# buggyyang/CDC_compression

Measured on AMD Instinct MI355X. Metric: decoded images/sec at 256x256, 500-step x-param, higher is better.
Workload: dtype f32 (f16x2 split products)

## Files before the change

### cdc_compression_amd/_lib.py

```python
import ctypes
import os
import subprocess

import numpy as np

_HERE = os.path.dirname(os.path.abspath(__file__))
LIB_PATH = os.environ.get("CDC_HIP_LIB") or os.path.join(_HERE, "libcdc_hip.so")

CDC_MEM_HOST, CDC_MEM_DEVICE = 0, 1
CDC_PRED_X, CDC_PRED_NOISE, CDC_PRED_NOISE_XTREE, CDC_PRED_V = 0, 1, 2, 3
CDC_CLIP_NONE, CDC_CLIP_ALL, CDC_CLIP_HALF = 0, 1, 2
CDC_MAX_LEVELS = 8
CDC_ELEM_F32, CDC_ELEM_U8 = 0, 1
CDC_FILL_EDGE, CDC_FILL_ZERO = 0, 1
CDC_METRIC_PSNR, CDC_METRIC_MSSSIM = 1, 2
CDC_TRACE_X0, CDC_TRACE_XT, CDC_TRACE_U8 = 1, 2, 4

_f = ctypes.POINTER(ctypes.c_float)
_i = ctypes.c_int
_vp = ctypes.c_void_p


class UnetConfig(ctypes.Structure):
    _fields_ = [("dim", ctypes.c_int32), ("channels", ctypes.c_int32),
# ... 162 lines not shown
    L.cdc_randn_host.argtypes = [u64p, _i, ctypes.c_int64, ctypes.c_uint32, ctypes.c_float, _vp]
    L.cdc_philox4x32_10.argtypes = [ctypes.POINTER(ctypes.c_uint32)] * 3
    i32p = ctypes.POINTER(ctypes.c_int32)
    L.cdc_set_noise_frames.argtypes = [H, i32p, _i]
    L.cdc_randn_framed.argtypes = [H, u64p, i32p, _i, _i, _i, _i, ctypes.c_uint32, ctypes.c_float, _vp, _i, _vp]
    L.cdc_randn_framed_host.argtypes = [u64p, i32p, _i, _i, _i, _i, ctypes.c_uint32, ctypes.c_float, _vp]
    L.cdc_tile_gather.argtypes = [H, _vp, _vp, i32p] + [_i] * 8 + [_vp]
    L.cdc_tile_blend.argtypes = [H, _vp, _vp, i32p, _i, i32p, _i, _vp] + [_i] * 14 + [_vp]
    L.cdc_prof_enable.argtypes = [H, _i]
    L.cdc_prof_name.argtypes = [_i]
    L.cdc_prof_name.restype = ctypes.c_char_p
    L.cdc_prof_get.argtypes = [H, _i, ctypes.POINTER(ctypes.c_double),
                               ctypes.POINTER(ctypes.c_int64), ctypes.POINTER(ctypes.c_double),
                               ctypes.POINTER(ctypes.c_double)]
    L.cdc_prof_reset.argtypes = [H]
    L.cdc_prof_num_ops.argtypes = [H]
    L.cdc_prof_op.argtypes = [H, _i, ctypes.POINTER(ctypes.c_char_p), ctypes.POINTER(ctypes.c_double),
                              ctypes.POINTER(ctypes.c_int64), ctypes.POINTER(ctypes.c_double)]
    L.cdc_op_conv2d.argtypes = [H, _vp, _vp, _vp, _vp] + [_i] * 9 + [_vp, _vp, _i, _vp, _vp]
    L.cdc_op_conv_transpose2d.argtypes = [H, _vp, _vp, _vp, _vp] + [_i] * 5
    L.cdc_op_chan_layernorm.argtypes = [H, _vp, _vp, _vp, _vp, _i, _i, _i]
    L.cdc_op_chan_layernorm_ex.argtypes = [H, _vp, _i, _vp, _vp, _i, _vp, _vp, _i, _vp, _vp, _vp, _i, _i, _i]
    L.cdc_op_ln_form.argtypes = [H, _i, _i, _i, _i, _i] + [ctypes.POINTER(_i)] * 4
    L.cdc_op_sum_slices.argtypes = [H, _vp, _i, _vp, _i, ctypes.c_longlong]
    L.cdc_op_linear_attention.argtypes = [H] + [_vp] * 7 + [_i] * 4
    L.cdc_op_stress.argtypes = [H, _i]
    L.cdc_op_stress_result.argtypes = [H, ctypes.POINTER(ctypes.c_int64), ctypes.POINTER(ctypes.c_int64)]
    L.cdc_probe_mfma_f16.argtypes = [_i, _i, _i, ctypes.POINTER(ctypes.c_double)]
    L.cdc_probe_hbm_copy.argtypes = [_i, ctypes.c_size_t, _i, ctypes.POINTER(ctypes.c_double)]
    _lib = L
# ... 11 lines not shown
           "cdc_entropy_encode", "cdc_entropy_peek", "cdc_entropy_set_limit", "cdc_entropy_decode", "cdc_get_range_faults",
           "cdc_get_nonfinite_results", "cdc_set_schedule_v", "cdc_probe_mfma_f16", "cdc_probe_hbm_copy",
           "cdc_op_stress", "cdc_op_stress_result", "cdc_enable_vbr", "cdc_set_bitrate_scale", "cdc_entropy_peek_bitrate_scale",
           "cdc_padded_size", "cdc_frame_pad", "cdc_frame_crop", "cdc_entropy_set_image_scale", "cdc_entropy_encode_image",
           "cdc_entropy_peek_image_size", "cdc_decode_seeded", "cdc_randn", "cdc_randn_host", "cdc_philox4x32_10",
           "cdc_distortion", "cdc_lpips_create", "cdc_lpips", "cdc_simple_encoder_create", "cdc_simple_ctxdec_create", "cdc_op_gdn",
           "cdc_op_gdn_workgroups", "cdc_op_chan_layernorm_ex", "cdc_op_ln_form", "cdc_op_sum_slices",
           "cdc_set_solver", "cdc_decode_solver", "cdc_solver_step", "cdc_op_solver_update", "cdc_op_ddim_update",
           "cdc_repeat_images", "cdc_decode_samples", "cdc_sample_moments", "cdc_sample_select",
           "cdc_set_trace", "cdc_trace_info", "cdc_trace_read", "cdc_op_trace_tap",
           "cdc_rate_map", "cdc_distortion_map", "cdc_set_rdo", "cdc_entropy_rate_sweep", "cdc_op_rdo_quantize",
           "cdc_price_cells", "cdc_set_rdo_map", "cdc_op_rdo_quantize_map",
           "cdc_set_noise_frames", "cdc_randn_framed", "cdc_randn_framed_host", "cdc_tile_gather", "cdc_tile_blend",
           "cdc_entropy_set_segments", "cdc_entropy_peek_segments", "cdc_entropy_decode_window",
           "cdc_entropy_set_hyper_groups", "cdc_entropy_peek_hyper_groups",
           "cdc_entropy_peek_partial", "cdc_entropy_decode_partial", "cdc_segment_mask"]


def handle_status(handle):
    if handle is None:
        return {"arith": None, "range_faults": 0, "nonfinite_results": 0}
    L = lib()
    return {"arith": int(L.cdc_get_arith(handle)), "range_faults": int(L.cdc_get_range_faults(handle)),
            "nonfinite_results": int(L.cdc_get_nonfinite_results(handle))}


def check(handle, rc):
    if rc != 0:
        msg = lib().cdc_last_error(handle)
        msg = msg.decode() if msg else ""
        if "must be multiples of" in msg:
# ... 90 lines not shown
```

### cdc_compression_amd/csrc/cdc_api.hip

```cpp
#include "cdc_state.h"
#include "rng.h"

namespace cdcapi {

std::string g_create_err;

int fail(cdc_handle *h, int code, const char *fmt, ...) {
    char buf[1024];
    va_list ap;
    va_start(ap, fmt);
    vsnprintf(buf, sizeof buf, fmt, ap);
    va_end(ap);
    if (h) h->err = buf; else g_create_err = buf;
    return code;
}

hipEvent_t get_event(cdc_handle *h) {
    if (!h->ev_free.empty()) { hipEvent_t e = h->ev_free.back(); h->ev_free.pop_back(); return e; }
    hipEvent_t e = nullptr;
    (void)hipEventCreate(&e);
    return e;
}

int resolve_pending(cdc_handle *h) {
// ... 38 lines not shown
        if (rc) return rc;
    }
    return CDC_OK;
}

int run_pre(cdc_handle *h, hipStream_t st) {
    for (const Op &op : h->pre_ops) {
        int rc = run_op(h, op, h->pB, st);
        if (rc) return rc;
    }
    return CDC_OK;
}

int run_unet(cdc_handle *h, hipStream_t st, int step, bool skip_combine) {
    for (const Op &op : h->ops) {
        if (skip_combine && op.get<CombineArgs>()) continue;
        int rc;
        if (op.get<TembArgs>() && (step >= 0 || step == -2)) {
            CopyArgs c = {h->d_shift_tab.p + (step >= 0 ? (size_t)step * h->shift_bs : 0), 0, h->shift, h->shift_bs, h->shift_bs};
            if (step == -2) { c.step = h->d_step; c.step_stride = h->shift_bs; }
            Op cop(op.prof, c, op.flops, op.bytes);
            cop.id = op.id;
            rc = run_op(h, cop, h->pB, st);
        } else {
            rc = run_op(h, op, h->pB, st);
        }
        if (rc) return rc;
    }
    return CDC_OK;
}
// ... 106 lines not shown
    return !no_guard && (h->arith == CDC_ARITH_F16X2 || h->in_retry);
}
int arm_range_guard(cdc_handle *h, hipStream_t st, bool always) {
    if (!always && !guard_enabled(h)) return CDC_OK;
    if (!h->d_fault) { void *p = nullptr; HIP_TRY(h, hipMalloc(&p, sizeof(int))); h->d_fault = (int *)p; h->weight_allocs.push_back(p); }
    HIP_TRY(h, hipMemsetAsync(h->d_fault, 0, sizeof(int), st));
    return CDC_OK;
}
int range_check(cdc_handle *h, const std::vector<GuardBuf> &bufs, int B, hipStream_t st) {
    if (!guard_enabled(h)) return CDC_OK;
    for (const GuardBuf &g : bufs)
        if (g.p && g.n > 0) HIP_TRY(h, cdc::nonfinite_launch(g.p, g.bs, g.n, B, h->d_fault, st));
    int fault = 0;
    HIP_TRY(h, hipMemcpyAsync(&fault, h->d_fault, sizeof(int), hipMemcpyDeviceToHost, st));
    HIP_TRY(h, hipStreamSynchronize(st));
    if (!fault) return CDC_OK;
    if (h->in_retry || h->arith != CDC_ARITH_F16X2) {
        ++h->nonfinite_results;
        if (h->in_retry) h->retry_futile = true;
        return CDC_OK;
    }
    ++h->range_faults;
    static bool warned = false;
    if (!warned) {
        warned = true;
        fprintf(stderr, "cdc_hip: a value left the fp16 range of CDC_ARITH_F16X2; the call is repeated in CDC_ARITH_BF16X3 and the handle stays "
                        "in that (slower, full-range) arithmetic -- see cdc_get_range_faults()\n");
    }
    int rc = cdc_set_arith(h, CDC_ARITH_BF16X3);
    return rc ? rc : kRangeRetry;
}

static int run_compressor(cdc_handle *h, const float *x, size_t n, int B, int mem, hipStream_t st) {
    int rc;
    if ((rc = stage_rate(h, nullptr, B, st))) return rc;
    if ((rc = copy_in(h, h->in_x, x, n, mem, st))) return rc;
    if ((rc = arm_range_guard(h, st, false))) return rc;
    h->prof_now = true;
    if ((rc = run_ops(h, h->pB, st))) return rc;
    std::vector<GuardBuf> outs;
    for (const Act &a : h->dec_outs) outs.push_back({a.p, a.bs(), (long long)a.C * a.H * a.W});
    return range_check(h, outs, B, st);
}

}

extern "C" {

const char *cdc_version(void) { return "cdc_hip 0.9 (gfx950; fp32-class convolutions from split fp16 / bf16 operands on the matrix cores)"; }

const char *cdc_last_error(const cdc_handle *h) { return h ? h->err.c_str() : g_create_err.c_str(); }

int cdc_create(const cdc_unet_config *cfg, int device, cdc_handle **out) {
    if (!cfg || !out) return fail(nullptr, CDC_ERR_INVALID, "null argument");
    if (cfg->dim <= 0 || cfg->n_dim_mults < 1 || cfg->n_dim_mults > CDC_MAX_LEVELS ||
        cfg->n_context_dim_mults < 0 || cfg->n_context_dim_mults > CDC_MAX_LEVELS || cfg->channels < 1)
        return fail(nullptr, CDC_ERR_INVALID, "bad cdc_unet_config");
// ... 3 lines not shown
    h->device = device;
    h->out_dim = cfg->out_dim > 0 ? cfg->out_dim : cfg->channels;
    h->dims.push_back(cfg->channels);
    for (int i = 0; i < cfg->n_dim_mults; ++i) h->dims.push_back(cfg->dim * cfg->dim_mults[i]);
    h->context_dims.push_back(cfg->context_channels);
    for (int i = 0; i < cfg->n_context_dim_mults; ++i)
        h->context_dims.push_back(cfg->dim * cfg->context_dim_mults[i]);
    h->n_res = cfg->n_dim_mults;
    build_manifest(h.get());
    *out = h.release();
    return CDC_OK;
}

void cdc_destroy(cdc_handle *h) {
    if (!h) return;
    if (!h->own_stream) { delete h; return; }
    (void)hipSetDevice(h->device);
    (void)hipDeviceSynchronize();
    free_program(h);
    free_pool(&h->weight_allocs);
    h->d_tab.release();
    h->d_tab_v.release();
    h->d_time_steps.release();
    h->d_shift_tab.release();
    h->seeds.dev.release();
    h->frames.dev.release();
    h->tile_meta.dev.release();
    h->d_stab.release();
    h->d_hist.release();
    h->d_rep_stage.release();
// ... 6 lines not shown
    for (hipEvent_t e : h->ev_free) (void)hipEventDestroy(e);
    if (h->gev_in) (void)hipEventDestroy(h->gev_in);
    if (h->gev_out) (void)hipEventDestroy(h->gev_out);
    if (h->graph_exec) (void)hipGraphExecDestroy(h->graph_exec);
    if (h->ev0) (void)hipEventDestroy(h->ev0);
    if (h->ev1) (void)hipEventDestroy(h->ev1);
    if (h->own_stream) (void)hipStreamDestroy(h->own_stream);
    delete h;
}

int cdc_set_arith(cdc_handle *h, int mode) {
    if (!h) return CDC_ERR_INVALID;
    if (mode != CDC_ARITH_BF16X3 && mode != CDC_ARITH_F16X2) return fail(h, CDC_ERR_INVALID, "arith mode %d", mode);
    if (mode != h->arith) {
        if (h->own_stream) { (void)hipSetDevice(h->device); (void)hipDeviceSynchronize(); }
        free_program(h);
        h->arith = mode;
    }
    return CDC_OK;
}

int cdc_get_arith(const cdc_handle *h) { return h ? h->arith : CDC_ERR_INVALID; }
int cdc_get_range_faults(const cdc_handle *h) { return h ? h->range_faults : CDC_ERR_INVALID; }
int cdc_get_nonfinite_results(const cdc_handle *h) { return h ? h->nonfinite_results : CDC_ERR_INVALID; }

int cdc_enable_vbr(cdc_handle *h) {
    if (!h) return CDC_ERR_INVALID;
    if (h->kind == HandleKind::Unet) return fail(h, CDC_ERR_INVALID, "variable bitrate needs a context-decoder, encoder or hyper-decoder handle");
    if (h->simple)
        return fail(h, CDC_ERR_INVALID, "variable bitrate: SimpleCompressor has no working VBR form in the reference");
// ... 826 lines not shown
}

int cdc_ddim_step(cdc_handle *h, const float *x_in, int i, const float *const *ctx, int n_ctx,
                  const float *noise, float eta, float *x_out, int B, int H, int W, int pred_mode,
                  int clip, int mem, void *stream) {
    if (!h) return CDC_ERR_INVALID;
    return no_throw(h, [&] { return sampler_step(h, false, x_in, noise, eta, i, ctx, n_ctx, x_out, nullptr, B, H, W, pred_mode, clip, mem, stream); });
}

int cdc_solver_step(cdc_handle *h, const float *x_in, const float *x0_prev_in, int i, const float *const *ctx, int n_ctx, float *x_out,
                    float *x0_out, int B, int H, int W, int pred_mode, int clip, int mem, void *stream) {
    if (!h) return CDC_ERR_INVALID;
    return no_throw(h, [&] { return sampler_step(h, true, x_in, x0_prev_in, 0.f, i, ctx, n_ctx, x_out, x0_out, B, H, W, pred_mode, clip, mem, stream); });
}

static int decode_impl(cdc_handle *h, const float *init, float gamma, const uint64_t *seeds, float eta, const float *const *ctx,
                       int n_ctx, float *out, int B, int H, int W, int pred_mode, int clip, int mem, void *stream, bool solver = false,
                       int rep = 0) {
    return with_range_guard(h, [&]() -> int {
        int rc = require_kind(h, HandleKind::Unet);
        if (rc) return rc;
        if ((rc = check_ready(h))) return rc;
        if ((rc = sampler_ready(h, pred_mode, clip, solver))) return rc;
        if (!out || !ctx) return fail(h, CDC_ERR_INVALID, "null argument");
        const bool traced = !h->trace_steps.empty();
        std::vector<int> slot_of;
        int n_slots = 0;
        if (traced) {
            if (rep) return fail(h, CDC_ERR_INVALID, "cdc_decode_samples: a trace is set (cdc_set_trace); a trajectory belongs to a single decode");
            if ((n_slots = trace_plan(h, B, H, W, &slot_of)) < 0) return n_slots;
        }
        if ((rc = build_program(h, B, H, W))) return rc;
        if ((rc = ensure_time_rows(h, B))) return rc;
        hipStream_t st = pick_stream(h, stream, mem);
        const size_t n = (size_t)B * h->cfg.channels * H * W;
        if (solver && (rc = h->d_hist.grow(h, n))) return rc;
        if ((rc = arm_range_guard(h, st, true))) return rc;
        if (solver) HIP_TRY(h, hipMemsetAsync(h->d_hist.p, 0, n * sizeof(float), st));
        const bool gen_init = seeds && !init && gamma != 0.f;
        const unsigned long long *dseeds = nullptr;
        const NoiseFrame *dframes = nullptr;
        bool fquad = false;
        if (seeds && (gen_init || eta != 0.f)) {
            if ((rc = h->seeds.stage(h, seeds, (size_t)B, st))) return rc;
            dseeds = h->seeds.dev.p;
            if (rep && !h->noise_frames.empty())
// ... 598 lines not shown
    return CDC_OK;
}
int cdc_prof_num_classes(void) { return PC_COUNT; }
const char *cdc_prof_name(int cls) { return (cls >= 0 && cls < PC_COUNT) ? kProfNames[cls] : ""; }
int cdc_prof_get(cdc_handle *h, int cls, double *ms, int64_t *launches, double *flops, double *bytes) {
    if (!h || cls < 0 || cls >= PC_COUNT) return CDC_ERR_INVALID;
    int rc = resolve_pending(h);
    if (rc) return rc;
    if (cls == 0 && getenv("CDC_PROF_OPS")) {
        for (size_t i = 0; i < h->op_ms.size(); ++i)
            if (h->op_n[i])
                fprintf(stderr, "[op %3zu] %8.3f ms  %7.1f TF  x%ld  %s\n", i, h->op_ms[i] / h->op_n[i],
                        h->op_flops[i] / (h->op_ms[i] / h->op_n[i] * 1e-3) / 1e12, h->op_n[i],
                        h->op_label[i].c_str());
    }
    if (ms) *ms = h->prof_ms[cls];
    if (launches) *launches = h->prof_launches[cls];
    if (flops) *flops = h->prof_flops[cls];
    if (bytes) *bytes = h->prof_bytes[cls];
    return CDC_OK;
}
int cdc_prof_num_ops(cdc_handle *h) { return h ? (int)h->op_ms.size() : CDC_ERR_INVALID; }
int cdc_prof_op(cdc_handle *h, int idx, const char **label, double *ms, int64_t *launches, double *flops) {
    if (!h || idx < 0 || idx >= (int)h->op_ms.size()) return CDC_ERR_INVALID;
    int rc = resolve_pending(h);
    if (rc) return rc;
    if (label) *label = h->op_label[idx].c_str();
    if (ms) *ms = h->op_ms[idx];
    if (launches) *launches = h->op_n[idx];
    if (flops) *flops = h->op_flops[idx];
    return CDC_OK;
}
int cdc_prof_reset(cdc_handle *h) {
    if (!h) return CDC_ERR_INVALID;
    (void)resolve_pending(h);
    std::fill(h->op_ms.begin(), h->op_ms.end(), 0.0);
    std::fill(h->op_n.begin(), h->op_n.end(), 0L);
    for (int i = 0; i < PC_COUNT; ++i) {
        h->prof_ms[i] = h->prof_flops[i] = h->prof_bytes[i] = 0;
        h->prof_launches[i] = 0;
    }
    return CDC_OK;
}

}
```

### cdc_compression_amd/csrc/cdc_planner.hip

```cpp
#include "cdc_state.h"

namespace cdcapi {

constexpr int kKsTarget = 1024;

struct Builder {
    cdc_handle *h;
    int B;
    std::vector<void *> *pool;
    int rc = CDC_OK;
    int planB = 0;
    int pb() const { return planB > 0 ? planB : B; }
    std::vector<Op> *cur = nullptr;

    void emit(Op op) {
        op.id = (int)h->op_ms.size();
        h->op_ms.push_back(0); h->op_n.push_back(0); h->op_flops.push_back(op.flops);
        const bool hoisted = cur == &h->pre_ops;
        char buf[160];
        std::visit([&](const auto &payload) { op_label(payload, buf, sizeof buf, hoisted); }, op.p);
        if (hoisted && !strstr(buf, " HOIST") && strlen(buf) + 7 < sizeof buf) strcat(buf, " HOIST");
        h->op_label.push_back(buf);
        (cur ? cur : &h->ops)->push_back(op);
    }
// ... 835 lines not shown
    }
};

void free_program(cdc_handle *h) {
    free_pool(&h->act_allocs);
    h->ops.clear();
    h->pre_ops.clear();
    h->op_ms.clear(); h->op_n.clear(); h->op_label.clear(); h->op_flops.clear();
    if (h->graph_exec) { (void)hipGraphExecDestroy(h->graph_exec); h->graph_exec = nullptr; }
    h->in_ctx.clear();
    h->taps.clear();
    h->dec_outs.clear();
    h->act_bytes = 0;
    h->pB = h->pH = h->pW = 0;
    h->p_batch1_plan = false;
    h->time_steps_B = 0;
    h->d_rate = nullptr;
    h->lp_res = nullptr;
}

static bool program_built(const cdc_handle *h, int B, int H, int W, bool batch1_plan = false) {
    return h->pB == B && h->pH == H && h->pW == W && h->p_batch1_plan == batch1_plan;
}
static int commit_program(cdc_handle *h, const Builder &bd, int H, int W, bool batch1_plan = false) {
    if (bd.rc) return bd.rc;
    h->pB = bd.B; h->pH = H; h->pW = W;
    h->p_batch1_plan = batch1_plan;
    return CDC_OK;
}

int build_program(cdc_handle *h, int B, int H, int W) {
    if (program_built(h, B, H, W)) return CDC_OK;
    free_program(h);
    const int n = h->n_res;
    const int down = 1 << (n - 1);
    if (H % down || W % down)
        return fail(h, CDC_ERR_INVALID, "H=%d, W=%d must be multiples of %d (%d downsamples)", H, W,
                    down, n - 1);
    Builder bd{h, B, &h->act_allocs};
    Act x = bd.input(h->cfg.channels, H, W);
    h->in_time = bd.dalloc(B);
    h->shift = bd.dalloc((size_t)B * h->shift_bs);
    h->xa = bd.dalloc((size_t)B * h->cfg.channels * H * W);
    h->xb = bd.dalloc((size_t)B * h->cfg.channels * H * W);
    h->noise_buf = bd.dalloc((size_t)B * h->cfg.channels * H * W);
    const int n_ctx = std::min(n - 1, (int)h->context_dims.size() - 1);
    for (int l = 0; l < n_ctx; ++l) h->in_ctx.push_back(bd.new_act(h->context_dims[l], H >> l, W >> l, false));
    if (bd.rc) return bd.rc;

    bd.emit(Op(PC_SMALL, TembArgs{h->in_time, h->tm_w0, h->tm_b0, h->tm_w2, h->tm_b2, h->cfg.dim, h->d_temb_layers, (int)h->rbs.size(),
                                  h->shift, h->shift_bs}));
    bd.tap("temb", h->shift, 1, 1, h->shift_bs);

    std::vector<Act> skips;
    size_t rbi = 0, ati = 0;
    for (int i = 0; i < n; ++i) {
        const int HWl = x.H * x.W;
        float *sm = bd.dalloc((size_t)B * HWl), *sr = bd.dalloc((size_t)B * HWl);
        const bool has_ctx = i < n_ctx;
        const std::string dn = "downs." + std::to_string(i);
        x = bd.resblock(h->rbs[rbi], x, has_ctx ? &h->in_ctx[i] : nullptr, nullptr, nullptr, Builder::SITE_RB_CHAIN,
                        bd.rb_reads_planes_only(h->rbs[rbi + 1], h->rbs[rbi].cout, x.H, x.W));
        ++rbi;
        h->taps[dn + ".0"] = x;
        x = bd.resblock(h->rbs[rbi++], x, nullptr, sm, sr);
        h->taps[dn + ".1"] = x;
        bd.tap(dn + ".1.stat_mean", sm, 1, x.H, x.W);
        bd.tap(dn + ".1.stat_rstd", sr, 1, x.H, x.W);
        const bool l0_planes = i == 0 && n > 1 && bd.pf_s2_would_plan(h->downs[0], x.H, x.W);
        bool skip_planes = false;
        if (i >= 1 && i < n - 1 && !dev_env("CDC_NO_PF_SKIP_PLANES")) {
            const ResBlockW &jrb = h->rbs[(size_t)2 * n + 2 + 2 * (n - 1 - i)];
// ... 670 lines not shown
```

### cdc_compression_amd/csrc/cdc_state.h

```cpp
#pragma once
#include <math.h>
#include <stdarg.h>
#include <stdio.h>
#include <stdlib.h>
#include <string.h>

#include <algorithm>
#include <map>
#include <memory>
#include <string>
#include <variant>
#include <vector>

#include "../../include/cdc_hip.h"
#include "cdc_internal.h"
#include "conv_ws_kernel.h"
#include "conv_ws1_kernel.h"
#include "entropy.h"

using namespace cdc;

namespace cdcapi {


// ... 277 lines not shown
    int op_stress_n = 0;
    long long op_stress_launches = 0, op_stress_differing = 0;
    bool prof = false;
    double prof_ms[PC_COUNT] = {0}, prof_flops[PC_COUNT] = {0}, prof_bytes[PC_COUNT] = {0};
    int64_t prof_launches[PC_COUNT] = {0};
    hipEvent_t ev0 = nullptr, ev1 = nullptr;
    struct Pending { hipEvent_t a, b; int cls; double flops, bytes; int id; };
    std::vector<double> op_ms;
    std::vector<long> op_n;
    std::vector<std::string> op_label;
    std::vector<double> op_flops;
    std::vector<Pending> pending;
    std::vector<hipEvent_t> ev_free;
    int prof_every = 1;
    bool prof_now = false;
};

namespace cdcapi {

extern std::string g_create_err;
int fail(cdc_handle *h, int code, const char *fmt, ...);

#define HIP_TRY(h, expr)                                                                        \
    do {                                                                                        \
        hipError_t e_ = (expr);                                                                 \
        if (e_ != hipSuccess)                                                                   \
            return fail(h, CDC_ERR_HIP, "%s failed: %s (%s:%d)", #expr, hipGetErrorString(e_),  \
                        __FILE__, __LINE__);                                                    \
    } while (0)

// ... 9 lines not shown
void add_attn_params(cdc_handle *h, const std::string &p, int c);
int down_in_channels(const cdc_handle *h, int ind);
void build_manifest(cdc_handle *h);
int upload(cdc_handle *h, const float *src, size_t n, float **dst, std::vector<void *> *pool);
const std::vector<float> &hostp(cdc_handle *h, const std::string &name);
int upload_param(cdc_handle *h, const std::string &name, float **dst);
int pack_conv(cdc_handle *h, const float *w, const float *bias, int CoutF, int CinF, int KH, int KW, int stride, int pad, bool transposed,
              ConvW *cw, std::vector<void *> *pool, int ci0 = 0, int ncin = 0, int co0 = 0, int ncout = 0);
int pack_named_conv(cdc_handle *h, const std::string &wname, const std::string &bname, int stride, int pad, bool transposed, ConvW *cw,
                    int ci0 = 0, int ncin = 0, int co0 = 0, int ncout = 0);
int pack_qkv_folded(cdc_handle *h, const float *wq, const float *g, const float *bln, int C, int co0, int nco, ConvW *cw, std::vector<void *> *pool);
int pack_kvctx(cdc_handle *h, const float *wq, const float *g, const float *bn, int c, AttnW *a, std::vector<void *> *pool);
void free_pool(std::vector<void *> *pool);
void free_program(cdc_handle *h);
int build_program(cdc_handle *h, int B, int H, int W);
int build_encoder_program(cdc_handle *h, int B, int H, int W);
int build_simple_encoder_program(cdc_handle *h, int B, int H, int W);
int build_hyperdec_program(cdc_handle *h, int B, int hh, int wh, bool batch1_plan = false);
int build_ctxdec_program(cdc_handle *h, int B, int hl, int wl);
int build_simple_ctxdec_program(cdc_handle *h, int B, int hl, int wl);
int build_lpips_program(cdc_handle *h, int pairs, int H, int W);
size_t lpips_pair_bytes(int H, int W);
void build_lpips_manifest(cdc_handle *h);
void build_compressor_manifest(cdc_handle *h);
int stage_rate(cdc_handle *h, const float *rates, int B, hipStream_t st);
hipEvent_t get_event(cdc_handle *h);
int resolve_pending(cdc_handle *h);
int run_op(cdc_handle *h, const Op &op, int B, hipStream_t st);
int run_ops(cdc_handle *h, int B, hipStream_t st);
int run_pre(cdc_handle *h, hipStream_t st);
int run_unet(cdc_handle *h, hipStream_t st, int step, bool skip_combine = false);
int copy_in(cdc_handle *h, float *dst, const float *src, size_t n, int mem, hipStream_t st);
int copy_out(cdc_handle *h, float *dst, const float *src, size_t n, int mem, hipStream_t st);
int stage_ctx(cdc_handle *h, const float *const *ctx, int n_ctx, int B, int mem, hipStream_t st);
int stage_ctx_repeated(cdc_handle *h, const float *const *ctx, int n_ctx, int B, int K, int mem, hipStream_t st);
int ensure_device(cdc_handle *h);
hipStream_t pick_stream(cdc_handle *h, void *stream, int mem);
int check_ready(cdc_handle *h);
int require_kind(cdc_handle *h, HandleKind kind);

bool guard_enabled(const cdc_handle *h);
int arm_range_guard(cdc_handle *h, hipStream_t st, bool always);
struct GuardBuf { const float *p; long long bs, n; };
constexpr int kRangeRetry = -10000;
int range_check(cdc_handle *h, const std::vector<GuardBuf> &bufs, int B, hipStream_t st);
struct RetryScope {
    cdc_handle *h;
    explicit RetryScope(cdc_handle *h_) : h(h_) { h->in_retry = true; h->retry_futile = false; }
    ~RetryScope() {
        h->in_retry = false;
        if (h->retry_futile) {
            h->retry_futile = false;
            if (h->range_faults > 0) --h->range_faults;
            (void)cdc_set_arith(h, CDC_ARITH_F16X2);
        }
    }
};
template <class F> int with_range_guard(cdc_handle *h, F &&body) {
    int rc = body();
    if (rc != kRangeRetry) return rc;
// ... 83 lines not shown
```

### cdc_compression_amd/csrc/cdc_weights.hip

```cpp
#include "cdc_state.h"

namespace cdcapi {

void add_param(cdc_handle *h, const std::string &name, std::vector<int64_t> shape, bool optional) {
    Param p;
    p.name = name;
    p.optional = optional;
    p.shape = std::move(shape);
    h->pindex[name] = (int)h->params.size();
    h->params.push_back(std::move(p));
}

void add_resblock_params(cdc_handle *h, const std::string &p, int cin, int cout, int k, bool with_mlp) {
    const int d = h->cfg.dim;
    if (with_mlp) {
        add_param(h, p + ".mlp.1.weight", {cout, d});
        add_param(h, p + ".mlp.1.bias", {cout});
    }
    add_param(h, p + ".block1.block.0.weight", {cout, cin, k, k});
    add_param(h, p + ".block1.block.0.bias", {cout});
    add_param(h, p + ".block1.block.1.g", {1, cout, 1, 1});
    add_param(h, p + ".block1.block.1.b", {1, cout, 1, 1});
    add_param(h, p + ".block2.block.0.weight", {cout, cout, 3, 3});
    add_param(h, p + ".block2.block.0.bias", {cout});
// ... 502 lines not shown
    pool->clear();
}


}

extern "C" {

int cdc_finalize_weights(cdc_handle *h) {
    if (!h) return CDC_ERR_INVALID;
    for (const Param &p : h->params)
        if (!p.loaded && !p.optional) return fail(h, CDC_ERR_STATE, "missing key \"%s\"", p.name.c_str());
    int rc = ensure_device(h);
    if (rc) return rc;
    HIP_TRY(h, hipDeviceSynchronize());
    free_program(h);
    free_pool(&h->weight_allocs);
    h->d_fault = nullptr; h->d_step = nullptr;
    h->rbs.clear(); h->attns.clear(); h->downs.clear(); h->ups.clear(); h->vbrs.clear(); h->gdns.clear();
    if (h->kind == HandleKind::Encoder) {
        const int n = (int)h->enc_dims.size() - 1;
        int shift_off = 0;
        for (int i = 0; h->simple && i < n; ++i) {
            const std::string p = "enc." + std::to_string(i);
            if (i < n - 1 && !gdn_supported(h->enc_dims[i + 1]))
                return fail(h, CDC_ERR_UNSUPPORTED, "GDN over %d channels: the kernel takes multiples of 16 from 16 to 256", h->enc_dims[i + 1]);
            ConvW dw;
            if ((rc = pack_named_conv(h, p + ".0.weight", p + ".0.bias", 2, 2, false, &dw))) return rc;
            h->downs.push_back(dw);
            if (i < n - 1 && (rc = pack_gdn(h, p + ".2", h->enc_dims[i + 1], false))) return rc;
// ... 195 lines not shown
```

### cdc_compression_amd/unet.py

```python
import ctypes

import numpy as np

from . import _lib


def _is_torch(t):
    return type(t).__module__.startswith("torch")


def _as_host_f32(t):
    if _is_torch(t):
        t = t.detach().cpu().numpy()
    return np.ascontiguousarray(t, dtype=np.float32)


class _Arg:

    def __init__(self, t, device_index):
        self.keep = None
        if _is_torch(t) and t.is_cuda:
            import torch
            if t.device.index != device_index:
                raise _lib.CdcError(f"tensor on cuda:{t.device.index}, model on cuda:{device_index}")
# ... 45 lines not shown
        self.dim_mults = tuple(dim_mults)
        self.context_dim_mults = tuple(context_dim_mults)
        self.embd_type = embd_type
        self.training = False
        dim_mults, context_dim_mults, out_dim = self.dim_mults, self.context_dim_mults, self.out_dim

        def config():
            cfg = _lib.UnetConfig()
            cfg.dim, cfg.channels, cfg.context_channels, cfg.out_dim = dim, channels, context_channels, out_dim
            cfg.n_dim_mults, cfg.n_context_dim_mults = len(dim_mults), len(context_dim_mults)
            for i, m in enumerate(dim_mults):
                cfg.dim_mults[i] = m
            for i, m in enumerate(context_dim_mults):
                cfg.context_dim_mults[i] = m
            return cfg
        self._lh = _lib.Handle("cdc_create", config, _lib.device_index_of(device))

    def _handle(self):
        return self._lh.ptr

    _h = property(lambda self: self._lh.raw)

    @_h.setter
    def _h(self, h):
        self._lh.raw = h

    _finalized = property(lambda self: self._lh.finalized)
    device_index = property(lambda self: self._lh.device_index)

    def status(self):
        return self._lh.status()

    @property
    def range_faults(self):
        return self.status()["range_faults"]

    def to(self, device):
        self._lh.move(_lib.device_index_of(device))
        return self

    def eval(self):
        self.training = False
        return self

    def manifest(self):
        return self._lh.manifest()

    def load_state_dict(self, state_dict, strict=True):
        names = [n for n, _ in self.manifest()]
        missing = [n for n in names if n not in state_dict]
# ... 47 lines not shown
```

### include/cdc_hip.h

```cpp
#ifndef CDC_HIP_H
#define CDC_HIP_H

#include <stddef.h>
#include <stdint.h>

#ifdef __cplusplus
extern "C" {
#endif

typedef struct cdc_handle cdc_handle;

typedef enum {
    CDC_OK = 0,
    CDC_ERR_INVALID = -1,
    CDC_ERR_STATE = -2,
    CDC_ERR_HIP = -3,
    CDC_ERR_UNSUPPORTED = -4,
    CDC_ERR_NOMEM = -5
} cdc_status;

enum { CDC_MEM_HOST = 0, CDC_MEM_DEVICE = 1 };
enum { CDC_PRED_X = 0, CDC_PRED_NOISE = 1, CDC_PRED_NOISE_XTREE = 2, CDC_PRED_V = 3 };
enum { CDC_CLIP_NONE = 0, CDC_CLIP_ALL = 1, CDC_CLIP_HALF = 2 };
enum { CDC_MAX_LEVELS = 8 };
// ... 215 lines not shown
int cdc_lpips(cdc_handle *h, const cdc_image_view *a, const cdc_image_view *b, int B, int H, int W, double *lpips ,
              double *layers , int mem_kind, void *stream);

int cdc_dequantize(cdc_handle *h, const float *x, const float *offset, float *out, long long n, int mem_kind,
                   void *stream);

int cdc_probe_mfma_f16(int device, int random_operands, int iters, double *tflops);
int cdc_probe_hbm_copy(int device, size_t bytes, int reps, double *gbytes_per_s);

int cdc_prof_enable(cdc_handle *h, int on);
int cdc_prof_num_classes(void);
const char *cdc_prof_name(int cls);
int cdc_prof_get(cdc_handle *h, int cls, double *ms, int64_t *launches, double *flops,
                 double *bytes);
int cdc_prof_reset(cdc_handle *h);
int cdc_prof_num_ops(cdc_handle *h);
int cdc_prof_op(cdc_handle *h, int idx, const char **label, double *ms, int64_t *launches, double *flops);


int cdc_op_conv2d(cdc_handle *h, const float *x, const float *w, const float *bias, float *y,
                  int B, int Cin, int H, int W, int Cout, int KH, int KW, int stride, int pad,
                  const float *ln_g, const float *ln_b, int relu, const float *shift,
                  const float *resid);
int cdc_op_conv_transpose2d(cdc_handle *h, const float *x, const float *w, const float *bias,
                            float *y, int B, int Cin, int H, int W, int Cout);
int cdc_op_chan_layernorm(cdc_handle *h, const float *x, const float *g, const float *b, float *y,
                          int B, int C, int HW);
int cdc_op_chan_layernorm_ex(cdc_handle *h, const float *x, int nparts, const float *g, const float *b, int relu, const float *shift,
                             const float *resid, int in_place, float *y, float *stat_mean, float *stat_rstd, int B, int C, int HW);
int cdc_op_ln_form(cdc_handle *h, int B, int C, int HW, int nparts, int aligned16, int *kind, int *width, int *np, int *img_major);
// ... 25 lines not shown
```

Measured before the change: 5.410.

## Split large-batch diffusion decode into two concurrent half-batch chains on twin streams

Adds a twin handle that shares weights and schedule tables with the main handle and runs half of the batch on its own stream. Each sampling step is issued on both streams so their kernels can overlap, mainly to fill the GPU during low-resolution U-Net stages and launch gaps. It is enabled by default only when the batch is at least 8 and the batch-times-pixels count is large, and can be forced or disabled via API or environment. In exchange it adds a second activation program's memory, cross-stream events and extra complexity in profiling and the range guard.

```diff
diff --git a/cdc_compression_amd/_lib.py b/cdc_compression_amd/_lib.py
--- a/cdc_compression_amd/_lib.py
+++ b/cdc_compression_amd/_lib.py
@@ -200,6 +200,8 @@
                                ctypes.POINTER(ctypes.c_int64), ctypes.POINTER(ctypes.c_double),
                                ctypes.POINTER(ctypes.c_double)]
     L.cdc_prof_reset.argtypes = [H]
+    L.cdc_set_decode_chains.argtypes = [H, _i]
+    L.cdc_decode_chains.argtypes = [H, _i, _i, _i]
     L.cdc_prof_num_ops.argtypes = [H]
     L.cdc_prof_op.argtypes = [H, _i, ctypes.POINTER(ctypes.c_char_p), ctypes.POINTER(ctypes.c_double),
                               ctypes.POINTER(ctypes.c_int64), ctypes.POINTER(ctypes.c_double)]
@@ -241,7 +243,8 @@
            "cdc_set_noise_frames", "cdc_randn_framed", "cdc_randn_framed_host", "cdc_tile_gather", "cdc_tile_blend",
            "cdc_entropy_set_segments", "cdc_entropy_peek_segments", "cdc_entropy_decode_window",
            "cdc_entropy_set_hyper_groups", "cdc_entropy_peek_hyper_groups",
-           "cdc_entropy_peek_partial", "cdc_entropy_decode_partial", "cdc_segment_mask"]
+           "cdc_entropy_peek_partial", "cdc_entropy_decode_partial", "cdc_segment_mask",
+           "cdc_set_decode_chains", "cdc_decode_chains"]
 
 
 def handle_status(handle):
diff --git a/cdc_compression_amd/csrc/cdc_api.hip b/cdc_compression_amd/csrc/cdc_api.hip
--- a/cdc_compression_amd/csrc/cdc_api.hip
+++ b/cdc_compression_amd/csrc/cdc_api.hip
@@ -76,6 +76,7 @@
 
 int run_unet(cdc_handle *h, hipStream_t st, int step, bool skip_combine) {
     for (const Op &op : h->ops) {
+        if (h->mark_ev && &op - h->ops.data() == h->trunk_op) HIP_TRY(h, hipEventRecord(h->mark_ev, st));
         if (skip_combine && op.get<CombineArgs>()) continue;
         int rc;
         if (op.get<TembArgs>() && (step >= 0 || step == -2)) {
@@ -212,6 +213,9 @@
     int fault = 0;
     HIP_TRY(h, hipMemcpyAsync(&fault, h->d_fault, sizeof(int), hipMemcpyDeviceToHost, st));
     HIP_TRY(h, hipStreamSynchronize(st));
+    return range_verdict(h, fault);
+}
+int range_verdict(cdc_handle *h, int fault) {
     if (!fault) return CDC_OK;
     if (h->in_retry || h->arith != CDC_ARITH_F16X2) {
         ++h->nonfinite_results;
@@ -239,6 +243,41 @@
     std::vector<GuardBuf> outs;
     for (const Act &a : h->dec_outs) outs.push_back({a.p, a.bs(), (long long)a.C * a.H * a.W});
     return range_check(h, outs, B, st);
+}
+
+void drop_twin(cdc_handle *h) {
+    if (!h || !h->twin) return;
+    cdc_handle *t = h->twin;
+    h->twin = nullptr;
+    cdc_destroy(t);
+}
+
+static void bind_twin_weights(cdc_handle *h, cdc_handle *t) {
+    t->cfg = h->cfg; t->arith = h->arith; t->dims = h->dims; t->context_dims = h->context_dims; t->n_res = h->n_res; t->out_dim = h->out_dim;
+    t->tm_w0 = h->tm_w0; t->tm_b0 = h->tm_b0; t->tm_w2 = h->tm_w2; t->tm_b2 = h->tm_b2;
+    t->rbs = h->rbs; t->attns = h->attns; t->downs = h->downs; t->ups = h->ups;
+    t->fin_g = h->fin_g; t->fin_b = h->fin_b; t->fin_conv = h->fin_conv; t->fin_bias = h->fin_bias; t->fin_P = h->fin_P;
+    t->d_temb_layers = h->d_temb_layers; t->shift_bs = h->shift_bs;
+    t->finalized = true;
+}
+static void bind_twin_tables(cdc_handle *h, cdc_handle *t) {
+    t->steps = h->steps; t->sched_gen = h->sched_gen; t->tab_v_gen = h->tab_v_gen; t->stab_sched_gen = h->stab_sched_gen; t->solver_gen = h->solver_gen;
+    t->d_tab = h->d_tab; t->d_tab_v = h->d_tab_v; t->d_time_steps = h->d_time_steps; t->d_shift_tab = h->d_shift_tab; t->d_stab = h->d_stab;
+    t->prof = h->prof; t->prof_every = h->prof_every; t->in_retry = h->in_retry;
+}
+
+static cdc_handle *twin_of(cdc_handle *h) {
+    if (h->twin) return h->twin;
+    cdc_handle *t = new cdc_handle;
+    t->is_twin = true;
+    t->device = h->device;
+    h->twin = t;
+    bool ok = ensure_device(t) == CDC_OK;
+    for (hipEvent_t *e : {&h->sp_fence, &h->sp_iter, &h->sp_mark, &t->sp_fence, &t->sp_iter})
+        if (ok && !*e) ok = hipEventCreateWithFlags(e, hipEventDisableTiming) == hipSuccess;
+    if (!ok) { (void)hipGetLastError(); h->err = "split decode: the twin's stream or events could not be created"; drop_twin(h); return nullptr; }
+    bind_twin_weights(h, t);
+    return t;
 }
 
 }
@@ -272,6 +311,11 @@
 
 void cdc_destroy(cdc_handle *h) {
     if (!h) return;
+    drop_twin(h);
+    if (h->is_twin) {
+        h->d_tab = {}; h->d_tab_v = {}; h->d_time_steps = {}; h->d_shift_tab = {}; h->d_stab = {};
+    }
+    for (hipEvent_t e : {h->sp_fence, h->sp_iter, h->sp_mark}) if (e) (void)hipEventDestroy(e);
     if (!h->own_stream) { delete h; return; }
     (void)hipSetDevice(h->device);
     (void)hipDeviceSynchronize();
@@ -308,6 +352,7 @@
     if (mode != CDC_ARITH_BF16X3 && mode != CDC_ARITH_F16X2) return fail(h, CDC_ERR_INVALID, "arith mode %d", mode);
     if (mode != h->arith) {
         if (h->own_stream) { (void)hipSetDevice(h->device); (void)hipDeviceSynchronize(); }
+        drop_twin(h);
         free_program(h);
         h->arith = mode;
     }
@@ -1164,6 +1209,89 @@
     return no_throw(h, [&] { return sampler_step(h, true, x_in, x0_prev_in, 0.f, i, ctx, n_ctx, x_out, x0_out, B, H, W, pred_mode, clip, mem, stream); });
 }
 
+static int decode_split(cdc_handle *h, const float *init, float gamma, const uint64_t *seeds, float eta, const float *const *ctx, int n_ctx,
+                        float *out, int B, int H, int W, int pred_mode, int clip, int mem, void *stream, bool solver) {
+    cdc_handle *const t = h->twin, *const hc[2] = {h, t};
+    const int Bc[2] = {(B + 1) / 2, B / 2}, row0[2] = {0, Bc[0]};
+    const size_t per = (size_t)h->cfg.channels * H * W, nc[2] = {Bc[0] * per, Bc[1] * per};
+    int rc;
+    if ((rc = ensure_time_rows(h, Bc[0]))) return rc;
+    bind_twin_tables(h, t);
+    if (n_ctx != (int)h->in_ctx.size()) return fail(h, CDC_ERR_INVALID, "expected %d context tensors, got %d", (int)h->in_ctx.size(), n_ctx);
+    const bool gen_init = seeds && !init && gamma != 0.f, use_seeds = seeds && (gen_init || eta != 0.f);
+    for (int k = 0; k < 2; ++k) {
+        if (solver && (rc = hc[k]->d_hist.grow(hc[k], nc[k]))) { h->err = hc[k]->err; return rc; }
+        if (use_seeds && (rc = hc[k]->seeds.dev.grow(hc[k], (size_t)Bc[k]))) { h->err = hc[k]->err; return rc; }
+    }
+    const hipStream_t st[2] = {pick_stream(h, stream, mem), t->own_stream};
+    HIP_TRY(h, hipEventRecord(h->sp_fence, st[0]));
+    HIP_TRY(h, hipStreamWaitEvent(st[1], h->sp_fence, 0));
+    const unsigned long long *dseeds[2] = {nullptr, nullptr};
+    auto chains = [&]() -> int {
+        int rc;
+        for (int k = 0; k < 2; ++k) {
+            cdc_handle *c = hc[k];
+            if ((rc = arm_range_guard(c, st[k], true))) return rc;
+            if (solver) HIP_TRY(c, hipMemsetAsync(c->d_hist.p, 0, nc[k] * sizeof(float), st[k]));
+            if (use_seeds) {
+                if ((rc = c->seeds.stage(c, seeds + row0[k], (size_t)Bc[k], st[k]))) return rc;
+                dseeds[k] = c->seeds.dev.p;
+            }
+            if (init) { if ((rc = copy_in(c, c->in_x, init + row0[k] * per, nc[k], mem, st[k]))) return rc; }
+            else if (gen_init) HIP_TRY(c, randn_fill_launch(dseeds[k], Bc[k], (long long)per, 0u, gamma, c->in_x, st[k]));
+            else HIP_TRY(c, hipMemsetAsync(c->in_x, 0, nc[k] * sizeof(float), st[k]));
+            std::vector<const float *> cx((size_t)n_ctx);
+            for (int l = 0; l < n_ctx; ++l) {
+                if (!ctx[l]) return fail(c, CDC_ERR_INVALID, "null context tensor %d", l);
+                cx[l] = ctx[l] + (size_t)row0[k] * (size_t)c->in_ctx[l].bs();
+            }
+            if ((rc = stage_ctx(c, cx.data(), n_ctx, Bc[k], mem, st[k]))) return rc;
+            c->prof_now = false;
+            if ((rc = run_pre(c, st[k]))) return rc;
+        }
+        const bool skew = decode_chains_skew() && h->trunk_op >= 0;
+        const int clip_c[2] = {clip == CDC_CLIP_HALF ? CDC_CLIP_ALL : clip, clip == CDC_CLIP_HALF ? CDC_CLIP_NONE : clip};
+        for (int i = h->steps - 1; i >= 0; --i) {
+            const bool first = i == h->steps - 1, prof_now = (i % h->prof_every) == 0, alone = h->prof && prof_now;
+            h->prof_now = t->prof_now = prof_now;
+            if (alone && !first) HIP_TRY(h, hipStreamWaitEvent(st[0], t->sp_iter, 0));
+            if (first && skew) h->mark_ev = h->sp_mark;
+            rc = sampler_on_device(h, solver, i, {nullptr, dseeds[0], nullptr, false}, eta, h->in_x, Bc[0], H, W, pred_mode, clip_c[0], st[0]);
+            h->mark_ev = nullptr;
+            if (rc) return rc;
+            if (alone) {
+                HIP_TRY(h, hipEventRecord(h->sp_iter, st[0]));
+                HIP_TRY(h, hipStreamWaitEvent(st[1], h->sp_iter, 0));
+            } else if (first && skew) HIP_TRY(h, hipStreamWaitEvent(st[1], h->sp_mark, 0));
+            if ((rc = sampler_on_device(t, solver, i, {nullptr, dseeds[1], nullptr, false}, eta, t->in_x, Bc[1], H, W, pred_mode, clip_c[1], st[1]))) return rc;
+            if (h->prof) HIP_TRY(t, hipEventRecord(t->sp_iter, st[1]));
+            if (alone) HIP_TRY(h, hipStreamWaitEvent(st[0], t->sp_iter, 0));
+        }
+        h->prof_now = t->prof_now = true;
+        return CDC_OK;
+    };
+    rc = chains();
+    hipError_t e = hipEventRecord(t->sp_fence, st[1]);
+    if (e == hipSuccess) e = hipStreamWaitEvent(st[0], t->sp_fence, 0);
+    if (rc) {
+        (void)hipStreamSynchronize(st[1]);
+        if (!t->err.empty()) { h->err = t->err; t->err.clear(); }
+        return rc;
+    }
+    HIP_TRY(h, e);
+    if (guard_enabled(h)) {
+        HIP_TRY(h, cdc::nonfinite_launch(h->in_x, 0, (long long)nc[0], 1, h->d_fault, st[0]));
+        HIP_TRY(h, cdc::nonfinite_launch(t->in_x, 0, (long long)nc[1], 1, h->d_fault, st[0]));
+        int fault[2] = {0, 0};
+        HIP_TRY(h, hipMemcpyAsync(&fault[0], h->d_fault, sizeof(int), hipMemcpyDeviceToHost, st[0]));
+        HIP_TRY(h, hipMemcpyAsync(&fault[1], t->d_fault, sizeof(int), hipMemcpyDeviceToHost, st[0]));
+        HIP_TRY(h, hipStreamSynchronize(st[0]));
+        if ((rc = range_verdict(h, fault[0] | fault[1]))) return rc;
+    }
+    if ((rc = copy_out(h, out, h->in_x, nc[0], mem, st[0]))) return rc;
+    return copy_out(h, out + nc[0], t->in_x, nc[1], mem, st[0]);
+}
+
 static int decode_impl(cdc_handle *h, const float *init, float gamma, const uint64_t *seeds, float eta, const float *const *ctx,
                        int n_ctx, float *out, int B, int H, int W, int pred_mode, int clip, int mem, void *stream, bool solver = false,
                        int rep = 0) {
@@ -1180,6 +1308,18 @@
             if (rep) return fail(h, CDC_ERR_INVALID, "cdc_decode_samples: a trace is set (cdc_set_trace); a trajectory belongs to a single decode");
             if ((n_slots = trace_plan(h, B, H, W, &slot_of)) < 0) return n_slots;
         }
+        if (decode_chains_rule(h, B, H, W, traced, !h->noise_frames.empty(), rep > 0, clip == CDC_CLIP_HALF) == 2) {
+            const int B0 = (B + 1) / 2;
+            cdc_handle *t = twin_of(h);
+            if (t && !(h->pB == B0 && h->pH == H && h->pW == W && !h->p_batch1_plan)) free_program(h);
+            if (t && (build_program(t, B - B0, H, W) != CDC_OK || build_program(h, B0, H, W) != CDC_OK)) {
+                (void)hipGetLastError();
+                free_program(t);
+                t = nullptr;
+            }
+            if (t) return decode_split(h, init, gamma, seeds, eta, ctx, n_ctx, out, B, H, W, pred_mode, clip, mem, stream, solver);
+        }
+        if (h->twin && h->twin->pB) free_program(h->twin);
         if ((rc = build_program(h, B, H, W))) return rc;
         if ((rc = ensure_time_rows(h, B))) return rc;
         hipStream_t st = pick_stream(h, stream, mem);
@@ -1808,10 +1948,12 @@
                         h->op_flops[i] / (h->op_ms[i] / h->op_n[i] * 1e-3) / 1e12, h->op_n[i],
                         h->op_label[i].c_str());
     }
-    if (ms) *ms = h->prof_ms[cls];
-    if (launches) *launches = h->prof_launches[cls];
-    if (flops) *flops = h->prof_flops[cls];
-    if (bytes) *bytes = h->prof_bytes[cls];
+    const cdc_handle *t = h->twin;
+    if (t && (rc = resolve_pending(h->twin))) { h->err = t->err; return rc; }
+    if (ms) *ms = h->prof_ms[cls] + (t ? t->prof_ms[cls] : 0.0);
+    if (launches) *launches = h->prof_launches[cls] + (t ? t->prof_launches[cls] : 0);
+    if (flops) *flops = h->prof_flops[cls] + (t ? t->prof_flops[cls] : 0.0);
+    if (bytes) *bytes = h->prof_bytes[cls] + (t ? t->prof_bytes[cls] : 0.0);
     return CDC_OK;
 }
 int cdc_prof_num_ops(cdc_handle *h) { return h ? (int)h->op_ms.size() : CDC_ERR_INVALID; }
@@ -1819,10 +1961,12 @@
     if (!h || idx < 0 || idx >= (int)h->op_ms.size()) return CDC_ERR_INVALID;
     int rc = resolve_pending(h);
     if (rc) return rc;
+    const cdc_handle *t = h->twin && h->twin->op_ms.size() == h->op_ms.size() ? h->twin : nullptr;
+    if (t && (rc = resolve_pending(h->twin))) { h->err = t->err; return rc; }
     if (label) *label = h->op_label[idx].c_str();
-    if (ms) *ms = h->op_ms[idx];
+    if (ms) *ms = h->op_ms[idx] + (t ? t->op_ms[idx] : 0.0);
     if (launches) *launches = h->op_n[idx];
-    if (flops) *flops = h->op_flops[idx];
+    if (flops) *flops = h->op_flops[idx] + (t ? t->op_flops[idx] : 0.0);
     return CDC_OK;
 }
 int cdc_prof_reset(cdc_handle *h) {
@@ -1834,7 +1978,20 @@
         h->prof_ms[i] = h->prof_flops[i] = h->prof_bytes[i] = 0;
         h->prof_launches[i] = 0;
     }
-    return CDC_OK;
-}
-
-}
+    return h->twin ? cdc_prof_reset(h->twin) : CDC_OK;
+}
+
+int cdc_set_decode_chains(cdc_handle *h, int n) {
+    if (!h) return CDC_ERR_INVALID;
+    int rc = require_kind(h, HandleKind::Unet);
+    if (rc) return rc;
+    if (n < 0 || n > 2) return fail(h, CDC_ERR_INVALID, "cdc_set_decode_chains: %d (0 the library's rule, 1 one chain, 2 two chains)", n);
+    h->decode_chains = n;
+    return CDC_OK;
+}
+int cdc_decode_chains(const cdc_handle *h, int B, int H, int W) {
+    if (!h) return CDC_ERR_INVALID;
+    return decode_chains_rule(h, B, H, W, !h->trace_steps.empty(), !h->noise_frames.empty(), false, false);
+}
+
+}
diff --git a/cdc_compression_amd/csrc/cdc_planner.hip b/cdc_compression_amd/csrc/cdc_planner.hip
--- a/cdc_compression_amd/csrc/cdc_planner.hip
+++ b/cdc_compression_amd/csrc/cdc_planner.hip
@@ -873,6 +873,7 @@
     h->act_bytes = 0;
     h->pB = h->pH = h->pW = 0;
     h->p_batch1_plan = false;
+    h->trunk_op = -1;
     h->time_steps_B = 0;
     h->d_rate = nullptr;
     h->lp_res = nullptr;
@@ -886,6 +887,33 @@
     h->pB = bd.B; h->pH = H; h->pW = W;
     h->p_batch1_plan = batch1_plan;
     return CDC_OK;
+}
+
+static int chains_env(bool *skew) {
+    const char *e = dev_env("CDC_DECODE_CHAINS");
+    if (!e) return 0;
+    if (skew && strchr(e, 's')) *skew = true;
+    if (skew && strchr(e, 'n')) *skew = false;
+    const int v = atoi(e);
+    return v == 1 || v == 2 ? v : 0;
+}
+constexpr bool kChainsSkewDefault = false;
+constexpr int kChainsMinBatch = 8;
+constexpr long long kChainsMinPixels = 1LL << 21;
+bool decode_chains_skew() {
+    bool skew = kChainsSkewDefault;
+    (void)chains_env(&skew);
+    return skew;
+}
+int decode_chains_rule(const cdc_handle *h, int B, int H, int W, bool traced, bool frames, bool samples, bool clip_half) {
+    if (!h || h->kind != HandleKind::Unet || h->is_twin || B < 2 || H < 1 || W < 1 || traced || frames || samples) return 1;
+    if (clip_half && (B & 1)) return 1;
+    const char *genv = getenv("CDC_GRAPH");
+    if (genv && atoi(genv) != 0) return 1;
+    int want = h->decode_chains;
+    if (want == 0) want = chains_env(nullptr);
+    if (want == 1 || want == 2) return want;
+    return B >= kChainsMinBatch && (long long)B * H * W >= kChainsMinPixels ? 2 : 1;
 }
 
 int build_program(cdc_handle *h, int B, int H, int W) {
@@ -915,6 +943,7 @@
     size_t rbi = 0, ati = 0;
     for (int i = 0; i < n; ++i) {
         const int HWl = x.H * x.W;
+        if (h->trunk_op < 0 && HWl <= 32 * 32) h->trunk_op = (int)h->ops.size();
         float *sm = bd.dalloc((size_t)B * HWl), *sr = bd.dalloc((size_t)B * HWl);
         const bool has_ctx = i < n_ctx;
         const std::string dn = "downs." + std::to_string(i);
diff --git a/cdc_compression_amd/csrc/cdc_state.h b/cdc_compression_amd/csrc/cdc_state.h
--- a/cdc_compression_amd/csrc/cdc_state.h
+++ b/cdc_compression_amd/csrc/cdc_state.h
@@ -315,6 +315,14 @@
     std::vector<hipEvent_t> ev_free;
     int prof_every = 1;
     bool prof_now = false;
+    cdc_handle *twin = nullptr;
+    bool is_twin = false;
+    int decode_chains = 0;
+    hipEvent_t sp_fence = nullptr;
+    hipEvent_t sp_iter = nullptr;
+    hipEvent_t sp_mark = nullptr;
+    int trunk_op = -1;
+    hipEvent_t mark_ev = nullptr;
 };
 
 namespace cdcapi {
@@ -354,6 +362,8 @@
 void free_pool(std::vector<void *> *pool);
 void free_program(cdc_handle *h);
 int build_program(cdc_handle *h, int B, int H, int W);
+int decode_chains_rule(const cdc_handle *h, int B, int H, int W, bool traced, bool frames, bool samples, bool clip_half);
+bool decode_chains_skew();
 int build_encoder_program(cdc_handle *h, int B, int H, int W);
 int build_simple_encoder_program(cdc_handle *h, int B, int H, int W);
 int build_hyperdec_program(cdc_handle *h, int B, int hh, int wh, bool batch1_plan = false);
@@ -378,12 +388,14 @@
 hipStream_t pick_stream(cdc_handle *h, void *stream, int mem);
 int check_ready(cdc_handle *h);
 int require_kind(cdc_handle *h, HandleKind kind);
+void drop_twin(cdc_handle *h);
 
 bool guard_enabled(const cdc_handle *h);
 int arm_range_guard(cdc_handle *h, hipStream_t st, bool always);
 struct GuardBuf { const float *p; long long bs, n; };
 constexpr int kRangeRetry = -10000;
 int range_check(cdc_handle *h, const std::vector<GuardBuf> &bufs, int B, hipStream_t st);
+int range_verdict(cdc_handle *h, int fault);
 struct RetryScope {
     cdc_handle *h;
     explicit RetryScope(cdc_handle *h_) : h(h_) { h->in_retry = true; h->retry_futile = false; }
diff --git a/cdc_compression_amd/csrc/cdc_weights.hip b/cdc_compression_amd/csrc/cdc_weights.hip
--- a/cdc_compression_amd/csrc/cdc_weights.hip
+++ b/cdc_compression_amd/csrc/cdc_weights.hip
@@ -540,6 +540,7 @@
     int rc = ensure_device(h);
     if (rc) return rc;
     HIP_TRY(h, hipDeviceSynchronize());
+    drop_twin(h);
     free_program(h);
     free_pool(&h->weight_allocs);
     h->d_fault = nullptr; h->d_step = nullptr;
diff --git a/cdc_compression_amd/unet.py b/cdc_compression_amd/unet.py
--- a/cdc_compression_amd/unet.py
+++ b/cdc_compression_amd/unet.py
@@ -83,7 +83,12 @@
             for i, m in enumerate(context_dim_mults):
                 cfg.context_dim_mults[i] = m
             return cfg
-        self._lh = _lib.Handle("cdc_create", config, _lib.device_index_of(device))
+        self._chains = 0
+
+        def setup(h):
+            if self._chains:
+                _lib.check(h, _lib.lib().cdc_set_decode_chains(h, self._chains))
+        self._lh = _lib.Handle("cdc_create", config, _lib.device_index_of(device), setup)
 
     def _handle(self):
         return self._lh.ptr
@@ -103,6 +108,14 @@
     @property
     def range_faults(self):
         return self.status()["range_faults"]
+
+    def set_decode_chains(self, n):
+        _lib.check(self._handle(), _lib.lib().cdc_set_decode_chains(self._handle(), int(n)))
+        self._chains = int(n)
+        return self
+
+    def decode_chains(self, B, H, W):
+        return int(_lib.lib().cdc_decode_chains(self._handle(), int(B), int(H), int(W)))
 
     def to(self, device):
         self._lh.move(_lib.device_index_of(device))
diff --git a/include/cdc_hip.h b/include/cdc_hip.h
--- a/include/cdc_hip.h
+++ b/include/cdc_hip.h
@@ -253,6 +253,9 @@
 int cdc_prof_get(cdc_handle *h, int cls, double *ms, int64_t *launches, double *flops,
                  double *bytes);
 int cdc_prof_reset(cdc_handle *h);
+
+int cdc_set_decode_chains(cdc_handle *h, int n);
+int cdc_decode_chains(const cdc_handle *h, int B, int H, int W);
 int cdc_prof_num_ops(cdc_handle *h);
 int cdc_prof_op(cdc_handle *h, int idx, const char **label, double *ms, int64_t *launches, double *flops);
 
```

Result: faster. 5.508, median of 6 (+1.8%).
